# JonasFrey96/Visual-Odom-Pipeline

Measured on AMD Instinct MI355X. Metric: frames/sec @1241x376, 2000 KLT pts, 10-frame BA window, higher is better.
Workload: dtype u8/i32 (KLT, Shi-Tomasi) + f64 (DLT, BA); 1 GPU; kitti_shaped_1241x376_2000pts_ba10; sequences_per_gpu=256, batched_contexts_per_gpu=1, distinct_image_sequences=8, tracked_points=jittered grid (SURVEY 8d's fallback), launch=plain, solves_stopped_by_cap=0, solves_cut_and_rerun=0

## Files before the change

include/vo_mi355x.h:

```cpp
#ifndef VO_MI355X_H
#define VO_MI355X_H

#include <stdint.h>

#ifdef __cplusplus
extern "C" {
#endif

#define VO_ABI_VERSION 4

enum {
  VO_OK = 0,
  VO_E_INVALID = -1,
  VO_E_HIP = -2,
  VO_E_NOMEM = -3,
  VO_E_STATE = -4,
  VO_E_CAPACITY = -5,
  VO_E_NUMERIC = -6
};

typedef struct vo_ctx vo_ctx;


typedef struct {
// ... 395 lines not shown
  int32_t ba_landmarks, ba_observations, ba_iters, ba_accepted, ba_status, ba_done;
  int32_t t_final;
  double  ba_cost0, ba_cost;
  double  H[12];
  double  H_final[12];
} vo_pipe_record;

enum { VO_PIPE_LOST = 1, VO_PIPE_CAPACITY = 2, VO_PIPE_GROUPS = 4 };
enum { VO_PIPE_TRACK = 1, VO_PIPE_POSE = 2, VO_PIPE_TRIANGULATE = 4, VO_PIPE_ADJUST = 8, VO_PIPE_DETECT = 16, VO_PIPE_ALL = 31,
       VO_PIPE_TRACK_CANDIDATES = 32, VO_PIPE_TRACK_LANDMARKS = 64,
       VO_PIPE_KEEP_FREE_LISTS = 128 };
#define VO_PIPE_INFLIGHT 4
#define VO_PIPE_HIST 32

enum { VO_PIPE_K_TFIRST = 0, VO_PIPE_K_TTOTAL, VO_PIPE_K_HISTLEN, VO_PIPE_K_UV, VO_PIPE_K_UVFIRST, VO_PIPE_K_HIST, VO_PIPE_L_TLATEST,
       VO_PIPE_L_P, VO_PIPE_CAND, VO_PIPE_LM_L, VO_PIPE_LM_K, VO_PIPE_LM_KSHARED, VO_PIPE_DEAD_L, VO_PIPE_DEAD_K, VO_PIPE_COUNTS,
       VO_PIPE_POSES, VO_PIPE_N_TABLES };

int32_t vo_pipe_default_params(vo_pipe_params* p);
int32_t vo_pipe_create(vo_ctx* ctx, const double* K, const vo_pipe_params* prm);
int32_t vo_pipe_table_bytes(vo_ctx* ctx, int32_t which, uint64_t* bytes);
int32_t vo_pipe_table_write(vo_ctx* ctx, int32_t which, const void* src);
int32_t vo_pipe_table_read(vo_ctx* ctx, int32_t which, void* dst);
int32_t vo_pipe_commit(vo_ctx* ctx);
int32_t vo_pipe_step(vo_ctx* ctx, int32_t frame_idx, int32_t stages);
int32_t vo_pipe_step_host(vo_ctx* ctx, const uint8_t* const* frames, int32_t stride, int32_t stages);
int32_t vo_pipe_fetch(vo_ctx* ctx, vo_pipe_record* rec );
int32_t vo_pipe_set_ba_budget(vo_ctx* ctx, int32_t budget);
int32_t vo_pipe_lists_bytes(vo_ctx* ctx, uint64_t* bytes);
int32_t vo_pipe_lists_read(vo_ctx* ctx, void* dst);
int32_t vo_pipe_rows_read(vo_ctx* ctx, int32_t kind, const int32_t* rows, int32_t n, void* out);
int32_t vo_pipe_inliers_read(vo_ctx* ctx, uint8_t* mask, int32_t n);

typedef struct {
  int32_t ba_kernels;
  int32_t ba_lanes;
  int32_t ba_threads;
  int32_t ba_pitch_pad;
  int32_t ba_chunks;
  int32_t ba_workgroups;
  int32_t ba_workgroup_cap;
  int32_t ba_fold;
  int32_t klt_waves;
  int32_t klt_pair;
  int32_t st_two_kernels;
  int32_t st_band_rows;
  int32_t st_separate_nms;
  int32_t st_keep_eig;
  int32_t st_host_limit;
  int32_t xcd_remap_off;
  int32_t gate_groups;
  int32_t reserve_cus;
  int32_t gather_workgroups;
  int32_t reserved[13];
} vo_tuning;
int32_t vo_get_tuning(vo_ctx* ctx, vo_tuning* out);
int32_t vo_set_tuning(vo_ctx* ctx, const vo_tuning* t);

int32_t vo_frame_step_resident(vo_ctx* ctx, int32_t frame_idx, int32_t n_pts, int32_t do_dlt, int32_t do_ba,
                               int32_t do_st, int32_t mask_radius, const vo_klt_params* klt,
                               const vo_st_params* st, const vo_ba_params* ba);
int32_t vo_frame_fetch(vo_ctx* ctx, int32_t n_pts, float* p, uint8_t* status, float* err, float* X4,
                       double* depth1, double* reproj, double* poses, double* points, vo_ba_stats* stats,
                       float* corners, int32_t* n_corners);
int32_t vo_frame_step_host(vo_ctx* ctx, const uint8_t* const* frames, int32_t stride, int32_t n_pts, int32_t do_dlt, int32_t do_ba,
                           int32_t do_st, int32_t mask_radius, const vo_klt_params* klt,
                           const vo_st_params* st, const vo_ba_params* ba);
int32_t vo_host_alloc(uint64_t bytes, void** out);
int32_t vo_host_free(void* p);
int32_t vo_set_graph_mode(vo_ctx* ctx, int32_t on);
int32_t vo_set_side_stream(vo_ctx* ctx, int32_t on);
int32_t vo_step_layout(vo_ctx* ctx, int32_t* layout, int32_t* gate_groups, int32_t* reserved_cus);

enum { VO_PROF_FRAME = 0, VO_PROF_KLT = 1, VO_PROF_ST = 2, VO_PROF_DLT = 3, VO_PROF_BA = 4, VO_PROF_CLAHE_LUT = 5, VO_PROF_CLAHE_APPLY = 6,
       VO_PROF_HOM_SOLVE = 7, VO_PROF_HOM_SCORE = 8, VO_PROF_HOM_SELECT = 9, VO_PROF_HOM_FINISH = 10, VO_PROF_ORB_PYRAMID = 11,
       VO_PROF_ORB_CANDIDATES = 12, VO_PROF_ORB_RETAIN = 13, VO_PROF_ORB_DESCRIBE = 14,
       VO_PROF_FUND_SOLVE = 15, VO_PROF_FUND_SCORE = 16, VO_PROF_FUND_SELECT = 17, VO_PROF_FUND_FINISH = 18,
       VO_PROF_GMATCH_FORWARD = 19, VO_PROF_GMATCH_REVERSE = 20, VO_PROF_GMATCH_ACCEPT = 21, VO_PROF_HPOSE = 22,
       VO_PROF_SIM3_SOLVE = 23, VO_PROF_SIM3_SCORE = 24, VO_PROF_SIM3_SELECT = 25, VO_PROF_SIM3_FINISH = 26,
       VO_PROF_COUNT = 27 };
int32_t vo_profile_enable(vo_ctx* ctx, int32_t region_mask);
int32_t vo_profile_read(vo_ctx* ctx, int32_t region, double* total_ms, int32_t* count);
int32_t vo_debug_cycles(vo_ctx* ctx, int32_t which, int64_t* out8);

#ifdef __cplusplus
}
#endif
#endif
```

visual-odom-pipeline_amd/csrc/vo_klt.hip:

```cpp
#include "vo_klt_lk.h"

#include <stdlib.h>
#include <string.h>

template <int WAVES>
__global__ void __launch_bounds__(64, WAVES) k_klt_track(klt_args A, const float* __restrict__ p0, float* __restrict__ p1,
                                                  uint8_t* __restrict__ status, float* __restrict__ err,
                                                  int32_t* __restrict__ iters, unsigned long long* __restrict__ dbg,
                                                  const int32_t* __restrict__ counts) {
  int pt = blockIdx.x, bseq = blockIdx.y;
  if (A.xcd_remap) {
    const unsigned id = blockIdx.y * gridDim.x + blockIdx.x;
    const unsigned q = id >> 3;
    bseq = (int)(id & 7u) + 8 * (int)(q / (unsigned)A.n);
    pt = (int)(q % (unsigned)A.n);
  }
  if (pt >= A.n) return;
  const int lane = threadIdx.x;
  if (iters) iters += (size_t)bseq * A.iters_seq;
  const bool dead = counts && pt >= counts[bseq];
  if (iters && lane < A.iters_stride && (dead || lane > A.top)) iters[pt * A.iters_stride + lane] = -1;
  if (dead) return;
  p0 = vo_seq(p0, A.slab_seq, bseq); p1 = vo_seq(p1, A.slab_seq, bseq);
  status = vo_seq(status, A.slab_seq, bseq); err = vo_seq(err, A.slab_seq, bseq);
// ... 241 lines not shown
  p->win = 31; p->max_level = 3; p->max_count = 30; p->epsilon = 0.03; p->min_eig_threshold = 1e-4f; p->_pad = 0;
  return VO_OK;
}

static float klt_min_eig_numerator(float thr, float c) {
  auto from_ord = [](int64_t k) {
    const uint32_t u = (k >= 0) ? (uint32_t)k : (0x80000000u | (uint32_t)(-k));
    float f; memcpy(&f, &u, 4); return f;
  };
  const int64_t inf = 0x7F800000ll;
  if (!(thr == thr)) return __builtin_nanf("");
  int64_t lo = -inf, hi = inf;
  { volatile float q = from_ord(lo) / c; if (q >= thr) return from_ord(lo); }
  { volatile float q = from_ord(hi) / c; if (!(q >= thr)) return from_ord(hi); }
  while (hi - lo > 1) {
    const int64_t mid = lo + (hi - lo) / 2;
    volatile float q = from_ord(mid) / c;
    if (q >= thr) hi = mid; else lo = mid;
  }
  return from_ord(hi);
}

int32_t vo_klt_make_args(vo_ctx* c, int n, const vo_klt_params* prm, klt_args& A) {
  VO_CHECK(c, c->n_pushed >= 2, VO_E_STATE, "need two pushed frames");
  VO_CHECK(c, n >= 0 && n <= c->max_pts, VO_E_CAPACITY, "n exceeds max_pts");
  VO_CHECK(c, prm && prm->win >= 3 && prm->win <= VO_MAX_WIN && (prm->win & 1), VO_E_INVALID, "win must be odd, 3..31");
  VO_CHECK(c, prm->max_level >= 0 && prm->max_level < VO_MAX_LEVELS, VO_E_INVALID, "bad max_level");
  if (n == 0) return VO_OK;
  const vo_frame& P = c->fr[c->cur ^ 1];
  const vo_frame& C = c->fr[c->cur];
  int top = 0;
  for (int l = 1; l <= c->top && l <= prm->max_level; l++) {
    if (c->lv[l].w <= prm->win || c->lv[l].h <= prm->win) break;
    top = l;
  }
  for (int l = 0; l <= top; l++) {
    A.lv[l].imgI = P.img[l]; A.lv[l].derI = reinterpret_cast<const uint32_t*>(P.der[l]); A.lv[l].imgJ = C.img[l];
    A.lv[l].seq_px = c->lvl_px[l];
    A.lv[l].w = c->lv[l].w; A.lv[l].h = c->lv[l].h; A.lv[l].pitch = c->lv[l].pitch;
  }
  A.top = top; A.win = prm->win;
  A.xcd_remap = (!c->tune.xcd_remap_off && c->batch % 8 == 0) ? 1 : 0;
  int mc = prm->max_count; if (mc < 0) mc = 0; if (mc > 100) mc = 100;
  double eps = prm->epsilon; if (eps < 0) eps = 0; if (eps > 10) eps = 10;
  A.max_count = mc; A.eps2 = eps * eps; A.n = n;
  A.min_eig_num = klt_min_eig_numerator(prm->min_eig_threshold, (float)(2 * prm->win * prm->win));
  A.eps_lo = (float)(A.eps2 * (1.0 - 1e-6)); A.eps_hi = (float)(A.eps2 * (1.0 + 1e-6));
  A.iters_stride = prm->max_level + 1;
  A.slab_seq = c->slab_seq; A.iters_seq = (size_t)c->max_pts * VO_MAX_LEVELS;
  c->iters_stride = A.iters_stride;
  return VO_OK;
}

static void klt_launch_plain(vo_ctx* c, const klt_launch_rows& L, const klt_args& A) {
  const int waves = c->tune.klt_waves > 0 ? c->tune.klt_waves : 6;
#define VO_KLT_LAUNCH(WV) hipLaunchKernelGGL(k_klt_track<WV>, dim3(L.n, c->batch), dim3(64), 0, L.q, A, L.p0, L.p1, L.status, L.err, c->d_iters, c->d_dbg, L.counts)
#ifdef VO_EXPERIMENTS
  const int pair = c->tune.klt_pair;
  if (pair) {
    const int npair = (L.n + 1) / 2;
#define VO_KLT_LAUNCH2(WV) hipLaunchKernelGGL(k_klt_track2<WV>, dim3(npair, c->batch), dim3(64), 0, L.q, A, L.p0, L.p1, L.status, L.err, c->d_iters, L.counts)
    if (pair == 3) VO_KLT_LAUNCH2(3); else if (pair == 5) VO_KLT_LAUNCH2(5); else VO_KLT_LAUNCH2(4);
#undef VO_KLT_LAUNCH2
  } else
#endif
  if (waves <= 4) VO_KLT_LAUNCH(4); else if (waves == 5) VO_KLT_LAUNCH(5); else VO_KLT_LAUNCH(6);
#undef VO_KLT_LAUNCH
}

int32_t vo_klt_enqueue(vo_ctx* c, hipStream_t q, int n, const vo_klt_params* prm, size_t off_in, size_t off_out, const int32_t* d_counts, unsigned form) {
  const bool fb = form & KLT_FORM_FB, seeded = form & KLT_FORM_SEEDED;
  c->fb.n = -1;
  c->guess.n = -1;
  klt_args A;
  { const int32_t r = vo_klt_make_args(c, n, prm, A); if (r != VO_OK) return r; }
  if (n == 0) { if (fb) c->fb.n = 0; return VO_OK; }
  if (seeded) VO_CHECK(c, c->guess.d, VO_E_STATE, "no guesses");
  klt_fb_args F;
  if (fb) {
    { const int32_t r = vo_fb_reserve(c); if (r != VO_OK) return r; }
    vo_klt_fb_make_args(c, A, F);
  }
  const klt_launch_rows L = {q, n, vo_slab<const float>(c, off_in), vo_slab<float>(c, off_out), vo_slab<uint8_t>(c, c->off_status),
                        vo_slab<float>(c, c->off_err), d_counts};
  {
    vo_prof_scope prof(c, q, VO_PROF_KLT);
    if (seeded) vo_klt_launch_seeded(c, L, A, fb ? &F : nullptr);
    else if (fb) vo_klt_launch_fb(c, L, A, F);
    else klt_launch_plain(c, L, A);
  }
  VO_HIP(c, hipGetLastError());
  if (fb) c->fb.n = n;
  return VO_OK;
}

static int32_t klt_track_sync(vo_ctx* c, unsigned form, const float* p0, const float* guess, int32_t n, const vo_klt_params* prm, float* p1,
                              uint8_t* status, float* err, float* p0r, float* fb_err, int32_t* iters) {
  if (!c) return VO_E_INVALID;
  const bool fb = form & KLT_FORM_FB, seeded = form & KLT_FORM_SEEDED;
  vo_klt_params def;
  if (!prm) { vo_klt_default_params(&def); prm = &def; }
  VO_CHECK(c, n >= 0 && n <= c->max_pts, VO_E_CAPACITY, "n exceeds max_pts");
  if (n == 0) return VO_OK;
  VO_CHECK(c, p0 && p1 && status && err && (!fb || (p0r && fb_err)), VO_E_INVALID, "null buffer");
  VO_HIP(c, hipSetDevice(c->device));
  { const int32_t rq = vo_quiesce_side(c); if (rq != VO_OK) return rq; }
  if (seeded) { const int32_t rg = vo_guess_reserve(c); if (rg != VO_OK) return rg; }
// ... 81 lines not shown
```

visual-odom-pipeline_amd/csrc/vo_klt_lk.h:

```cpp
#pragma once
#include "vo_internal.h"

#define W_BITS 14

struct klt_level_args {
  const uint8_t* imgI;
  const uint32_t* derI;
  const uint8_t* imgJ;
  size_t seq_px;
  int w, h, pitch;
};

struct klt_args {
  klt_level_args lv[VO_MAX_LEVELS];
  size_t slab_seq;
  size_t iters_seq;
  int top, win, max_count, n, iters_stride;
  int xcd_remap;
  float min_eig_num;
  float eps_lo, eps_hi;
  double eps2;
};

struct klt_fb_args {
  klt_level_args bw[VO_MAX_LEVELS];
  size_t fb_seq;
  size_t off_err, off_ok;
  float max_err;
};

typedef uint32_t u32x3 __attribute__((ext_vector_type(3)));
__device__ __forceinline__ __amdgpu_buffer_rsrc_t klt_rsrc(const void* base) {
  return __builtin_amdgcn_make_buffer_rsrc(const_cast<void*>(base), 0, -1, 0x00020000);
}

__device__ __forceinline__ uint32_t row_next(uint32_t v, int lane) {
  return (uint32_t)__builtin_amdgcn_ds_bpermute(((lane + 16) & 63) << 2, (int)v);
}

__device__ __forceinline__ int wave_sum_i32(int v) {
  v += __builtin_amdgcn_update_dpp(0, v, 0x111 , 0xf, 0xf, false);
  v += __builtin_amdgcn_update_dpp(0, v, 0x112 , 0xf, 0xf, false);
  v += __builtin_amdgcn_update_dpp(0, v, 0x114 , 0xf, 0xf, false);
  v += __builtin_amdgcn_update_dpp(0, v, 0x118 , 0xf, 0xf, false);
  v += __builtin_amdgcn_update_dpp(0, v, 0x142 , 0xa, 0xf, false);
  v += __builtin_amdgcn_update_dpp(0, v, 0x143 , 0xc, 0xf, false);
  return __builtin_amdgcn_readlane(v, 63);
}

__device__ __forceinline__ float wave_sum_exact_f32(int v) {
  const int lo = wave_sum_i32(v & 0xFFFF);
  const int hi = wave_sum_i32(v >> 16);
  return (float)((double)hi * 65536.0 + (double)lo);
}
// ... 52 lines not shown
  const int w1 = klt_rows_sum(z >> 16);
  la = __builtin_amdgcn_readlane(w0, 0); lb = __builtin_amdgcn_readlane(w0, 1);
  lc = __builtin_amdgcn_readlane(w0, 2); hc = __builtin_amdgcn_readlane(w0, 3);
  ha = __builtin_amdgcn_readlane(w1, 0); hb = __builtin_amdgcn_readlane(w1, 1);
}

__device__ __forceinline__ float klt_combine(int hi, int lo) {
  if ((unsigned)(hi + 16384) < 32768u) return (float)(hi * 65536 + lo);
  return (float)((double)hi * 65536.0 + (double)lo);
}

__device__ __forceinline__ int klt_round(float x) { return __float_as_int(x + 12582912.f) - 0x4B400000; }

__device__ __forceinline__ void lk_weights(float a, float b, uint32_t& wt, uint32_t& wb) {
  const uint32_t r00 = (uint32_t)__float_as_int((1.f - a) * (1.f - b) * (float)(1 << W_BITS) + 12582912.f);
  const uint32_t r01 = (uint32_t)__float_as_int(a * (1.f - b) * (float)(1 << W_BITS) + 12582912.f);
  const uint32_t r10 = (uint32_t)__float_as_int((1.f - a) * b * (float)(1 << W_BITS) + 12582912.f);
  const uint32_t iw11 = (uint32_t)(1 << W_BITS) + 3u * 0x4B400000u - (r00 + r01 + r10);
  wt = __builtin_amdgcn_perm(r01, r00, 0x05040100u);
  wb = __builtin_amdgcn_perm(iw11, r10, 0x05040100u);
}

__device__ __forceinline__ float uniform_f(float v) {
  return __int_as_float(__builtin_amdgcn_readfirstlane(__float_as_int(v)));
}

typedef short s16x2 __attribute__((ext_vector_type(2)));

__device__ __forceinline__ int dot2(uint32_t a, uint32_t b, int c) {
  return __builtin_amdgcn_sdot2(__builtin_bit_cast(s16x2, a), __builtin_bit_cast(s16x2, b), c, false);
}
__device__ __forceinline__ int dot2k(uint32_t a, uint32_t b, int c) {
  return __builtin_amdgcn_sdot2(__builtin_bit_cast(s16x2, a), __builtin_bit_cast(s16x2, b), c, true);
}
__device__ __forceinline__ uint32_t pack_lo(uint32_t a, uint32_t b) { return __builtin_amdgcn_perm(b, a, 0x05040100u); }
__device__ __forceinline__ uint32_t pack_hi(uint32_t a, uint32_t b) { return __builtin_amdgcn_perm(b, a, 0x07060302u); }
__device__ __forceinline__ uint32_t bytes01(uint32_t t) { return __builtin_amdgcn_perm(0u, t, 0x0c010c00u); }
__device__ __forceinline__ uint32_t bytes12(uint32_t t) { return __builtin_amdgcn_perm(0u, t, 0x0c020c01u); }
__device__ __forceinline__ uint32_t pk_sub(uint32_t a, uint32_t b) {
  return __builtin_bit_cast(uint32_t, __builtin_bit_cast(s16x2, a) - __builtin_bit_cast(s16x2, b));
}
__device__ __forceinline__ uint32_t pk_abs(uint32_t a) {
  const s16x2 v = __builtin_bit_cast(s16x2, a);
  return __builtin_bit_cast(uint32_t, __builtin_elementwise_max(v, -v));
}

__device__ __forceinline__ uint32_t sample2(uint32_t T, uint32_t B, uint32_t wt, uint32_t wb) {
  const int s0 = dot2(bytes01(B), wb, dot2k(bytes01(T), wt, 1 << (W_BITS - 5 - 1)));
  const int s1 = dot2(bytes12(B), wb, dot2k(bytes12(T), wt, 1 << (W_BITS - 5 - 1)));
  typedef unsigned short u16x2 __attribute__((ext_vector_type(2)));
  const u16x2 h = __builtin_bit_cast(u16x2, __builtin_amdgcn_perm((uint32_t)s1, (uint32_t)s0, 0x06050201u));
  return __builtin_bit_cast(uint32_t, h >> (unsigned short)(W_BITS - 5 - 8));
}

__device__ __forceinline__ uint32_t deriv1(uint32_t top, uint32_t bot, uint32_t wt, uint32_t wb) {
  return (uint32_t)dot2(bot, wb, dot2k(top, wt, 1 << (W_BITS + 1)));
}

template <bool SEEDED = false>
__device__ __forceinline__ void klt_lk_point(const klt_args& A, const klt_level_args (&lv)[VO_MAX_LEVELS], int bseq, int pt, int lane,
                                             float p0x, float p0y, int32_t* iters, unsigned long long* dbgk,
                                             float& outx, float& outy, int& st, float& errv, float gx = 0.f, float gy = 0.f) {
  VO_STAMP(dbgk, 0);
  const int cp = lane & 15, r = lane >> 4;
  const int win = A.win;
  const float half = (float)(win - 1) * 0.5f;
  const float FLT_SCALE = 1.f / (float)(1 << 20);

  outx = 0.f; outy = 0.f;
  st = 1;
  errv = 0.f;

  const uint32_t colmask = ((2 * cp < win) ? 0x0000FFFFu : 0u) | ((2 * cp + 1 < win) ? 0xFFFF0000u : 0u);
  const uint32_t colones = colmask & 0x00010001u;
  const uint32_t colsel = (0x07060302u & colmask) | (0x0c0c0c0cu & ~colmask);

  for (int level = A.top; level >= 0; level--) {
    klt_level_args L = lv[level];
    L.imgI += (size_t)bseq * L.seq_px; L.derI += (size_t)bseq * L.seq_px; L.imgJ += (size_t)bseq * L.seq_px;
    const float scale = __int_as_float((127 - level) << 23);
    float prevx = p0x * scale, prevy = p0y * scale;
    float nextx, nexty;
    if (level == A.top) {
      if (SEEDED) { nextx = gx * scale; nexty = gy * scale; }
      else { nextx = prevx; nexty = prevy; }
    }
    else { nextx = outx * 2.f; nexty = outy * 2.f; }
    outx = nextx; outy = nexty;
    int n_it = -1;

    prevx -= half; prevy -= half;
    const float fpx = floorf(prevx), fpy = floorf(prevy);
    const int ipx = (int)fpx, ipy = (int)fpy;
    if (ipx < -win || ipx >= L.w || ipy < -win || ipy >= L.h) {
      if (level == 0) { st = 0; errv = 0.f; }
      if (iters && lane == 0) iters[pt * A.iters_stride + level] = n_it;
      continue;
    }
    const uint32_t lane_off = (uint32_t)(8 * r * L.pitch + 2 * cp);
    uint32_t wt, wb;
    lk_weights(prevx - fpx, prevy - fpy, wt, wb);

    uint32_t tI[8], tX[8], tY[8];
    {
      uint32_t T[8], D0[8], D1[8], D2[8];
      const uint32_t uo = (uint32_t)(ipy + VO_PAD) * (uint32_t)L.pitch + (uint32_t)(ipx + VO_PAD);
      const __amdgpu_buffer_rsrc_t rI = klt_rsrc(L.imgI), rD = klt_rsrc(L.derI);
#pragma unroll
      for (int s = 0; s < 8; s++) {
        const uint32_t o = uo + (uint32_t)s * (uint32_t)L.pitch;
        T[s] = __builtin_amdgcn_raw_buffer_load_b32(rI, (int)lane_off, (int)o, 0);
        const u32x3 d3 = __builtin_amdgcn_raw_buffer_load_b96(rD, (int)(lane_off * 4u), (int)(o * 4u), 0);
        D0[s] = d3[0]; D1[s] = d3[1]; D2[s] = d3[2];
      }
      const uint32_t T8 = row_next(T[0], lane), D08 = row_next(D0[0], lane), D18 = row_next(D1[0], lane), D28 = row_next(D2[0], lane);
      int a11 = 0, a12 = 0, a22 = 0;
#pragma unroll
      for (int s = 0; s < 8; s++) {
        const uint32_t B = (s < 7) ? T[(s + 1) & 7] : T8;
        const uint32_t E0 = (s < 7) ? D0[(s + 1) & 7] : D08;
        const uint32_t E1 = (s < 7) ? D1[(s + 1) & 7] : D18;
        const uint32_t E2 = (s < 7) ? D2[(s + 1) & 7] : D28;
        tI[s] = sample2(T[s], B, wt, wb);
        const uint32_t x0 = deriv1(pack_lo(D0[s], D1[s]), pack_lo(E0, E1), wt, wb);
        const uint32_t y0 = deriv1(pack_hi(D0[s], D1[s]), pack_hi(E0, E1), wt, wb);
        const uint32_t x1 = deriv1(pack_lo(D1[s], D2[s]), pack_lo(E1, E2), wt, wb);
        const uint32_t y1 = deriv1(pack_hi(D1[s], D2[s]), pack_hi(E1, E2), wt, wb);
        const uint32_t sel = (8 * r + s < win) ? colsel : 0x0c0c0c0cu;
        const uint32_t xp = __builtin_amdgcn_perm(x1, x0, sel), yp = __builtin_amdgcn_perm(y1, y0, sel);
        tX[s] = xp; tY[s] = yp;
        a11 = s ? dot2(xp, xp, a11) : dot2k(xp, xp, 0);
        a12 = s ? dot2(xp, yp, a12) : dot2k(xp, yp, 0);
        a22 = s ? dot2(yp, yp, a22) : dot2k(yp, yp, 0);
      }
      float A11, A12, A22;
      {
        int l11, h11, l12, h12, l22, h22;
        wave_sum3_wide(a11, a12, a22, lane, l11, h11, l12, h12, l22, h22);
        A11 = klt_combine(h11, l11) * FLT_SCALE; A12 = klt_combine(h12, l12) * FLT_SCALE; A22 = klt_combine(h22, l22) * FLT_SCALE;
      }
      if (level == A.top) VO_STAMP(dbgk, 1);
      float D = A11 * A22 - A12 * A12;
      const float num = A22 + A11 - sqrtf((A11 - A22) * (A11 - A22) + 4.f * A12 * A12);
      if (num < A.min_eig_num || D < 1.1920929e-07f) {
        if (level == 0) st = 0;
        if (iters && lane == 0) iters[pt * A.iters_stride + level] = n_it;
        continue;
      }
      D = 1.f / D;

      nextx -= half; nexty -= half;
      const __amdgpu_buffer_rsrc_t rJ = klt_rsrc(L.imgJ);
      float pdx = 0.f, pdy = 0.f;
      int j = 0;
      for (; j < A.max_count; j++) {
        const float fnx = floorf(nextx), fny = floorf(nexty);
        const int inx = (int)fnx, iny = (int)fny;
        if (inx < -win || inx >= L.w || iny < -win || iny >= L.h) {
          if (level == 0) st = 0;
          break;
        }
        uint32_t jt, jb;
        lk_weights(nextx - fnx, nexty - fny, jt, jb);
        uint32_t Tj[8];
        const uint32_t uj = (uint32_t)(iny + VO_PAD) * (uint32_t)L.pitch + (uint32_t)(inx + VO_PAD);
#pragma unroll
        for (int s = 0; s < 8; s++) Tj[s] = __builtin_amdgcn_raw_buffer_load_b32(rJ, (int)lane_off, (int)(uj + (uint32_t)s * (uint32_t)L.pitch), 0);
        const uint32_t Tj8 = row_next(Tj[0], lane);
        int b1 = 0, b2 = 0;
#pragma unroll
        for (int s = 0; s < 8; s++) {
          const uint32_t B = (s < 7) ? Tj[(s + 1) & 7] : Tj8;
          const uint32_t d = pk_sub(sample2(Tj[s], B, jt, jb), tI[s]);
          b1 = s ? dot2(d, tX[s], b1) : dot2k(d, tX[0], 0);
          b2 = s ? dot2(d, tY[s], b2) : dot2k(d, tY[0], 0);
        }
        int l1, h1, l2, h2;
        wave_sum2_wide(b1, b2, lane, l1, h1, l2, h2);
        const float fb1 = klt_combine(h1, l1) * FLT_SCALE;
        const float fb2 = klt_combine(h2, l2) * FLT_SCALE;
        const float dx = (A12 * fb2 - A22 * fb1) * D;
        const float dy = (A12 * fb1 - A11 * fb2) * D;
        nextx += dx; nexty += dy;
        outx = nextx + half; outy = nexty + half;
        const float d2 = dx * dx + dy * dy;
        bool conv;
        if (d2 < A.eps_lo) conv = true;
        else if (d2 > A.eps_hi) conv = false;
        else conv = (double)dx * (double)dx + (double)dy * (double)dy <= A.eps2;
        if (conv) { j++; break; }
        if (j > 0 && fabsf(dx + pdx) <= 0.01f && fabsf(dy + pdy) <= 0.01f) {
          outx -= dx * 0.5f; outy -= dy * 0.5f;
          j++;
          break;
        }
        pdx = dx; pdy = dy;
        if (level == A.top && j == 0) VO_STAMP(dbgk, 2);
      }
      n_it = j;
      if (level == A.top) VO_STAMP(dbgk, 3);
      if (level == 1) VO_STAMP(dbgk, 4);
      if (iters && lane == 0) iters[pt * A.iters_stride + level] = n_it;

      if (st && level == 0) {
        const float nx = outx - half, ny = outy - half;
        const float fnx = floorf(nx), fny = floorf(ny);
        const int inx = (int)fnx, iny = (int)fny;
        if (inx < -win || inx >= L.w || iny < -win || iny >= L.h) {
          st = 0;
        } else {
          uint32_t jt, jb;
          lk_weights(nx - fnx, ny - fny, jt, jb);
          uint32_t Tj[8];
          const uint32_t uj = (uint32_t)(iny + VO_PAD) * (uint32_t)L.pitch + (uint32_t)(inx + VO_PAD);
#pragma unroll
          for (int s = 0; s < 8; s++) Tj[s] = __builtin_amdgcn_raw_buffer_load_b32(rJ, (int)lane_off, (int)(uj + (uint32_t)s * (uint32_t)L.pitch), 0);
          const uint32_t Tj8 = row_next(Tj[0], lane);
          int e = 0;
#pragma unroll
          for (int s = 0; s < 8; s++) {
            const uint32_t B = (s < 7) ? Tj[(s + 1) & 7] : Tj8;
            const uint32_t d = pk_abs(pk_sub(sample2(Tj[s], B, jt, jb), tI[s]));
            const uint32_t ones = (8 * r + s < win) ? colones : 0u;
            e = s ? dot2(d, ones, e) : dot2k(d, ones, 0);
          }
          const int ierr = wave_sum_i32(e);
          errv = (float)ierr * 1.f / (float)(32 * win * win);
        }
      }
    }
  }
  VO_STAMP(dbgk, 5);
}

int32_t vo_klt_enqueue(vo_ctx* c, hipStream_t q, int n, const vo_klt_params* prm, size_t off_in, size_t off_out, const int32_t* d_counts, unsigned form);
int32_t vo_klt_make_args(vo_ctx* c, int n, const vo_klt_params* prm, klt_args& A);
void vo_klt_fb_make_args(const vo_ctx* c, const klt_args& A, klt_fb_args& F);

struct klt_launch_rows {
  hipStream_t q;
  int n;
  const float* p0; float* p1; uint8_t* status; float* err;
  const int32_t* counts;
};
void vo_klt_launch_fb(vo_ctx* c, const klt_launch_rows& L, const klt_args& A, const klt_fb_args& F);
void vo_klt_launch_seeded(vo_ctx* c, const klt_launch_rows& L, const klt_args& A, const klt_fb_args* F);

inline hipError_t iters_d2h(vo_ctx* c, int32_t* h, int n, int levels) {
  return rows_d2h(c, h, c->d_iters, sizeof(int32_t) * (size_t)c->max_pts * VO_MAX_LEVELS, sizeof(int32_t) * (size_t)n * levels);
}
```

visual-odom-pipeline_amd/csrc/vo_step.hip:

```cpp
#include "vo_internal.h"

#include <stdlib.h>
#include <string.h>

#include <mutex>
#include <vector>
#include <stdio.h>
static std::mutex g_trace_mu;
static std::vector<hipEvent_t> g_tr, g_ta, g_tb;
static void trace_push(std::vector<hipEvent_t>& v, hipStream_t st, size_t cap) {
  std::lock_guard<std::mutex> lk(g_trace_mu);
  if (v.size() >= cap) return;
  hipEvent_t e;
  if (hipEventCreate(&e) != hipSuccess) return;
  (void)hipEventRecord(e, st);
  v.push_back(e);
}
extern "C" void vo_debug_step_trace_dump(int first_step, int n_steps) {
  std::lock_guard<std::mutex> lk(g_trace_mu);
  for (size_t i = 2 * (size_t)(first_step < 0 ? 0 : first_step); i + 3 < g_tr.size() && i + 3 < g_ta.size() && i + 3 < g_tb.size() && i < 2 * (size_t)(first_step + n_steps); i += 2) {
    float d = 0, gap = 0, a0 = 0, a1 = 0;
    (void)hipEventElapsedTime(&d, g_tr[i], g_tr[i + 1]);
    (void)hipEventElapsedTime(&gap, g_tr[i + 1], g_tr[i + 2]);
    (void)hipEventElapsedTime(&a0, g_tr[i], g_ta[i + 2]);
// ... 392 lines not shown
    if (c->tune.gate_groups) groups = c->tune.gate_groups > 0 ? c->tune.gate_groups : 0;
    if (c->tune.reserve_cus) reserve = c->tune.reserve_cus > 0 ? c->tune.reserve_cus : 0;
  }
  c->ba_wide_groups = groups;
  c->ba_wide_recorded = false;
  c->layout_suspended = false;
  return vo_main_stream_reserve(c, reserve);
}

static int32_t pipelined_setup(vo_ctx* c) {
  hipEvent_t (*const pairs[4])[2] = {&c->ev_ba_wide, &c->ev_ba, &c->ev_pub, &c->ev_copy1};
  hipStream_t st = nullptr; hipEvent_t ev[8] = {};
  VO_HIP(c, hipSetDevice(c->device));
  hipError_t e = hipStreamCreateWithFlags(&st, hipStreamNonBlocking);
  for (int i = 0; i < 8 && e == hipSuccess; i++) e = hipEventCreateWithFlags(&ev[i], hipEventDisableTiming);
  if (e != hipSuccess) {
    for (hipEvent_t x : ev) if (x) (void)hipEventDestroy(x);
    if (st) (void)hipStreamDestroy(st);
    VO_HIP(c, e);
  }
  for (int i = 0; i < 8; i++) (*pairs[i / 2])[i % 2] = ev[i];
  c->stream3 = st;
  return VO_OK;
}

extern "C" int32_t vo_set_side_stream(vo_ctx* c, int32_t on) {
  if (!c) return VO_E_INVALID;
  VO_CHECK(c, c->steps_enq == c->steps_fetched && !vo_pipe_busy(c), VO_E_STATE, "fetch the steps in flight before switching the stream layout");
  if (on == 2 && !c->stream3) { const int32_t rs = pipelined_setup(c); if (rs != VO_OK) return rs; }
  c->side_stream = (on == 2) ? 2 : (on ? 1 : 0);
  return step_layout_apply(c);
}

extern "C" int32_t vo_get_tuning(vo_ctx* c, vo_tuning* out) {
  if (!c || !out) return VO_E_INVALID;
  *out = c->tune;
  return VO_OK;
}

extern "C" int32_t vo_set_tuning(vo_ctx* c, const vo_tuning* t) {
  if (!c || !t) return VO_E_INVALID;
  VO_CHECK(c, c->steps_enq == c->steps_fetched && !vo_pipe_busy(c), VO_E_STATE, "fetch the steps in flight before changing the tuning");
  VO_CHECK(c, (t->ba_kernels >= 0 && t->ba_kernels <= 2) && (t->ba_lanes == 0 || t->ba_lanes == 8 || t->ba_lanes == 16) &&
              (t->ba_threads == 0 || t->ba_threads == 256 || t->ba_threads == 512 || t->ba_threads == 1024) && t->ba_pitch_pad >= 0 && t->ba_pitch_pad <= 64 &&
              t->ba_chunks >= 0 && t->ba_workgroups >= 0 && t->ba_workgroup_cap >= 0 && t->ba_fold >= 0 && t->ba_fold <= 2 &&
              (t->klt_waves == 0 || (t->klt_waves >= 4 && t->klt_waves <= 6)) && t->st_band_rows >= 0 && t->gate_groups >= -1 && t->reserve_cus >= -1 &&
              t->reserve_cus < 256, VO_E_INVALID, "field out of range");
#ifndef VO_EXPERIMENTS
  VO_CHECK(c, t->klt_pair == 0, VO_E_INVALID, "klt_pair needs a build with -DVO_EXPERIMENTS");
#else
  VO_CHECK(c, t->klt_pair == 0 || (t->klt_pair >= 3 && t->klt_pair <= 5), VO_E_INVALID, "klt_pair: 3, 4 or 5");
#endif
  VO_CHECK(c, t->gather_workgroups >= 0 && t->gather_workgroups <= 65536, VO_E_INVALID, "gather_workgroups out of range");
  for (int k = 0; k < 13; k++) VO_CHECK(c, t->reserved[k] == 0, VO_E_INVALID, "reserved fields must be 0");
  VO_HIP(c, hipSetDevice(c->device));
  { const int32_t rq = vo_quiesce_side(c); if (rq != VO_OK) return rq; }
  c->tune = *t;
  for (auto& g : c->step_graphs) if (g.second) (void)hipGraphExecDestroy(g.second);
  c->step_graphs.clear();
  return step_layout_apply(c);
}

extern "C" int32_t vo_step_layout(vo_ctx* c, int32_t* layout, int32_t* gate_groups, int32_t* reserved_cus) {
  if (!c) return VO_E_INVALID;
  if (layout) *layout = c->side_stream;
  if (gate_groups) *gate_groups = c->ba_wide_groups;
  if (reserved_cus) *reserved_cus = c->stream_reserve;
  return VO_OK;
}

extern "C" int32_t vo_set_graph_mode(vo_ctx* c, int32_t on) {
  if (!c) return VO_E_INVALID;
  VO_CHECK(c, c->steps_enq == c->steps_fetched && !vo_pipe_busy(c), VO_E_STATE, "fetch the steps in flight before switching the launch mode");
  c->use_graph = on ? 1 : 0;
  { const int32_t rr = step_layout_apply(c); if (rr != VO_OK) return rr; }
  return VO_OK;
}
```

visual-odom-pipeline_amd/vo_mi355x/_lib.py:

```python
import ctypes as C
import os

import numpy as np

_HERE = os.path.dirname(os.path.abspath(__file__))
PKG_ROOT = os.path.dirname(_HERE)
LIB_PATH = os.environ.get("VO_MI355X_LIB") or os.path.join(PKG_ROOT, "lib", "libvo_mi355x.so")
CSRC_DIR = os.path.join(PKG_ROOT, "csrc")

VO_OK = 0
ERRORS = {-1: "VO_E_INVALID", -2: "VO_E_HIP", -3: "VO_E_NOMEM", -4: "VO_E_STATE", -5: "VO_E_CAPACITY",
          -6: "VO_E_NUMERIC"}


class VoError(RuntimeError):
    def __init__(self, code, msg):
        super().__init__("%s (%d): %s" % (ERRORS.get(code, "VO_E_?"), code, msg))
        self.code = code


class KltParams(C.Structure):
    _fields_ = [("win", C.c_int32), ("max_level", C.c_int32), ("max_count", C.c_int32),
                ("epsilon", C.c_double), ("min_eig_threshold", C.c_float), ("_pad", C.c_int32)]


class SubpixParams(C.Structure):
    _fields_ = [("win_x", C.c_int32), ("win_y", C.c_int32), ("zero_x", C.c_int32), ("zero_y", C.c_int32), ("max_count", C.c_int32),
                ("_pad", C.c_int32), ("epsilon", C.c_double)]


class BriefParams(C.Structure):
    _fields_ = [("n_bits", C.c_int32), ("_pad", C.c_int32), ("reserved", C.c_int32 * 6)]


class StParams(C.Structure):
    _fields_ = [("max_corners", C.c_int32), ("block_size", C.c_int32), ("quality_level", C.c_double),
                ("min_distance", C.c_double), ("use_harris", C.c_int32), ("fast_threshold", C.c_int32), ("harris_k", C.c_double)]


LOSSES = {"huber": 0, "linear": 1, "soft_l1": 2, "cauchy": 3, "arctan": 4}


def loss_code(loss):
    if callable(loss):
        raise NotImplementedError("a callable loss is not supported by the HIP bundle adjustment; use one of %s" % sorted(LOSSES))
    if loss not in LOSSES:
        raise ValueError("loss must be one of %s, got %r" % (sorted(LOSSES), loss))
    return LOSSES[loss]


class BaParams(C.Structure):
    _fields_ = [("max_iters", C.c_int32), ("loss", C.c_int32), ("ftol", C.c_double), ("xtol", C.c_double),
                ("gtol", C.c_double), ("lambda0", C.c_double), ("huber_delta", C.c_double), ("lambda_min", C.c_double)]


TUNING_FIELDS = ("ba_kernels", "ba_lanes", "ba_threads", "ba_pitch_pad", "ba_chunks", "ba_workgroups", "ba_workgroup_cap", "ba_fold", "klt_waves", "klt_pair",
                 "st_two_kernels", "st_band_rows", "st_separate_nms", "st_keep_eig", "st_host_limit", "xcd_remap_off", "gate_groups", "reserve_cus",
                 "gather_workgroups")


class Tuning(C.Structure):
    _fields_ = [(k, C.c_int32) for k in TUNING_FIELDS] + [("reserved", C.c_int32 * 13)]


class PnpParams(C.Structure):
    _fields_ = [("reproj_err", C.c_double), ("confidence", C.c_double), ("max_iters", C.c_int32), ("seed", C.c_int32)]


class PnpStats(C.Structure):
    _fields_ = [("cost", C.c_double), ("n_inliers", C.c_int32), ("hypotheses", C.c_int32), ("best", C.c_int32),
                ("status", C.c_int32)]


class EssParams(C.Structure):
    _fields_ = [("threshold", C.c_double), ("prob", C.c_double), ("distance_thresh", C.c_double), ("max_iters", C.c_int32),
                ("seed", C.c_int32)]


class EssStats(C.Structure):
    _fields_ = [("n_inliers", C.c_int32), ("n_good", C.c_int32), ("hypotheses", C.c_int32), ("best", C.c_int32),
                ("status", C.c_int32), ("_pad", C.c_int32)]


class HomParams(C.Structure):
    _fields_ = [("threshold", C.c_double), ("confidence", C.c_double), ("max_iters", C.c_int32), ("seed", C.c_int32),
                ("refine_iters", C.c_int32), ("_pad", C.c_int32)]


class HomStats(C.Structure):
    _fields_ = [("cost", C.c_double), ("n_inliers", C.c_int32), ("hypotheses", C.c_int32), ("best", C.c_int32),
                ("status", C.c_int32), ("lm_iters", C.c_int32), ("_pad", C.c_int32)]


class FundParams(C.Structure):
    _fields_ = [("threshold", C.c_double), ("confidence", C.c_double), ("max_iters", C.c_int32), ("seed", C.c_int32),
                ("refit", C.c_int32), ("_pad", C.c_int32)]


class FundStats(C.Structure):
    _fields_ = [("cost", C.c_double), ("n_inliers", C.c_int32), ("hypotheses", C.c_int32), ("best", C.c_int32),
                ("status", C.c_int32), ("n_roots", C.c_int32), ("models", C.c_int32)]


class Sim3Params(C.Structure):
    _fields_ = [("threshold", C.c_double), ("confidence", C.c_double), ("max_iters", C.c_int32), ("seed", C.c_int32),
                ("with_scale", C.c_int32), ("refit", C.c_int32)]


class Sim3Stats(C.Structure):
    _fields_ = [("cost", C.c_double), ("n_inliers", C.c_int32), ("hypotheses", C.c_int32), ("best", C.c_int32),
                ("status", C.c_int32), ("degenerate", C.c_int32), ("refit", C.c_int32)]


class HposeParams(C.Structure):
    _fields_ = [("ratio", C.c_double), ("threshold", C.c_double), ("hint", C.c_double * 3), ("min_off", C.c_int32), ("use_hint", C.c_int32)]
# ... 234 lines not shown
```

Before: 47600 frames/s.

## Cache KLT target-window rows in LDS across iterations within same integer cell

Adds a KLT tracking kernel variant that gathers the 9 rows of the target image window into LDS as byte-pair expansions and reuses them across Lucas-Kanade iterations while the integer patch position stays unchanged. Global buffer loads are reissued only when the wave-uniform cell changes. The variant is on by default through a tuning field when no wave or pair override is set. It is meant to cut repeated global loads and byte unpacking per iteration, at the cost of LDS traffic, a shared buffer per block, and asm pins that constrain scheduling.

Result: faster. 49240 frames/s (median of 6 runs) (+3.4%).

```diff
diff --git a/include/vo_mi355x.h b/include/vo_mi355x.h
--- a/include/vo_mi355x.h
+++ b/include/vo_mi355x.h
@@ -471,7 +471,8 @@
   int32_t gate_groups;
   int32_t reserve_cus;
   int32_t gather_workgroups;
-  int32_t reserved[13];
+  int32_t klt_reuse;
+  int32_t reserved[12];
 } vo_tuning;
 int32_t vo_get_tuning(vo_ctx* ctx, vo_tuning* out);
 int32_t vo_set_tuning(vo_ctx* ctx, const vo_tuning* t);
diff --git a/visual-odom-pipeline_amd/csrc/vo_klt.hip b/visual-odom-pipeline_amd/csrc/vo_klt.hip
--- a/visual-odom-pipeline_amd/csrc/vo_klt.hip
+++ b/visual-odom-pipeline_amd/csrc/vo_klt.hip
@@ -317,7 +317,10 @@
   return VO_OK;
 }
 
+#define KLT_REUSE_RULE 1
 static void klt_launch_plain(vo_ctx* c, const klt_launch_rows& L, const klt_args& A) {
+  const bool rule = KLT_REUSE_RULE && c->tune.klt_waves == 0 && c->tune.klt_pair == 0;
+  if (c->tune.klt_reuse > 0 || (c->tune.klt_reuse == 0 && rule)) { vo_klt_launch_reuse(c, L, A); return; }
   const int waves = c->tune.klt_waves > 0 ? c->tune.klt_waves : 6;
 #define VO_KLT_LAUNCH(WV) hipLaunchKernelGGL(k_klt_track<WV>, dim3(L.n, c->batch), dim3(64), 0, L.q, A, L.p0, L.p1, L.status, L.err, c->d_iters, c->d_dbg, L.counts)
 #ifdef VO_EXPERIMENTS
diff --git a/visual-odom-pipeline_amd/csrc/vo_klt_lk.h b/visual-odom-pipeline_amd/csrc/vo_klt_lk.h
--- a/visual-odom-pipeline_amd/csrc/vo_klt_lk.h
+++ b/visual-odom-pipeline_amd/csrc/vo_klt_lk.h
@@ -1,5 +1,7 @@
 #pragma once
 #include "vo_internal.h"
+
+#include <limits.h>
 
 #define W_BITS 14
 
@@ -158,12 +160,40 @@
   const u16x2 h = __builtin_bit_cast(u16x2, __builtin_amdgcn_perm((uint32_t)s1, (uint32_t)s0, 0x06050201u));
   return __builtin_bit_cast(uint32_t, h >> (unsigned short)(W_BITS - 5 - 8));
 }
+__device__ __forceinline__ uint2 sample2_gather(uint32_t T) { return make_uint2(bytes01(T), bytes12(T)); }
+__device__ __forceinline__ uint32_t sample2_combine(uint2 t, uint2 b, uint32_t wt, uint32_t wb) {
+  const int s0 = dot2(b.x, wb, dot2k(t.x, wt, 1 << (W_BITS - 5 - 1)));
+  const int s1 = dot2(b.y, wb, dot2k(t.y, wt, 1 << (W_BITS - 5 - 1)));
+  typedef unsigned short u16x2 __attribute__((ext_vector_type(2)));
+  const u16x2 h = __builtin_bit_cast(u16x2, __builtin_amdgcn_perm((uint32_t)s1, (uint32_t)s0, 0x06050201u));
+  return __builtin_bit_cast(uint32_t, h >> (unsigned short)(W_BITS - 5 - 8));
+}
+
+__device__ __forceinline__ char* klt_rows_lds() {
+  __shared__ uint2 rows[9 * 64];
+  return reinterpret_cast<char*>(rows);
+}
+__device__ __forceinline__ uint2 klt_row_read(const char* rows, uint32_t ab, int k) {
+  return *reinterpret_cast<const uint2*>(rows + ab + (uint32_t)k * 512u);
+}
+__device__ __forceinline__ void klt_rows_fetch(char* rows, uint32_t ab, __amdgpu_buffer_rsrc_t rJ, uint32_t lane_off, uint32_t uo, uint32_t pitch, int lane) {
+  uint32_t Tj[8];
+#pragma unroll
+  for (int s = 0; s < 8; s++) Tj[s] = __builtin_amdgcn_raw_buffer_load_b32(rJ, (int)lane_off, (int)(uo + (uint32_t)s * pitch), 0);
+  const uint32_t Tj8 = row_next(Tj[0], lane);
+#pragma unroll
+  for (int k = 0; k < 9; k++) {
+    *reinterpret_cast<uint2*>(rows + ab + (uint32_t)k * 512u) = sample2_gather(k < 8 ? Tj[k & 7] : Tj8);
+  }
+}
+#define KLT_ROWS_PIN(ab, acc) asm volatile("" : "+v"(ab), "+v"(acc))
+#define KLT_ROWS_OPAQUE(v) asm volatile("" : "+v"(v))
 
 __device__ __forceinline__ uint32_t deriv1(uint32_t top, uint32_t bot, uint32_t wt, uint32_t wb) {
   return (uint32_t)dot2(bot, wb, dot2k(top, wt, 1 << (W_BITS + 1)));
 }
 
-template <bool SEEDED = false>
+template <bool SEEDED = false, bool REUSE = false>
 __device__ __forceinline__ void klt_lk_point(const klt_args& A, const klt_level_args (&lv)[VO_MAX_LEVELS], int bseq, int pt, int lane,
                                              float p0x, float p0y, int32_t* iters, unsigned long long* dbgk,
                                              float& outx, float& outy, int& st, float& errv, float gx = 0.f, float gy = 0.f) {
@@ -180,6 +210,9 @@
   const uint32_t colmask = ((2 * cp < win) ? 0x0000FFFFu : 0u) | ((2 * cp + 1 < win) ? 0xFFFF0000u : 0u);
   const uint32_t colones = colmask & 0x00010001u;
   const uint32_t colsel = (0x07060302u & colmask) | (0x0c0c0c0cu & ~colmask);
+  char* rows = nullptr;
+  uint32_t rows_ab = 0;
+  if constexpr (REUSE) { rows = klt_rows_lds(); rows_ab = (uint32_t)lane * 8u; }
 
   for (int level = A.top; level >= 0; level--) {
     klt_level_args L = lv[level];
@@ -258,6 +291,7 @@
       nextx -= half; nexty -= half;
       const __amdgpu_buffer_rsrc_t rJ = klt_rsrc(L.imgJ);
       float pdx = 0.f, pdy = 0.f;
+      int cellx = INT_MIN, celly = INT_MIN;
       int j = 0;
       for (; j < A.max_count; j++) {
         const float fnx = floorf(nextx), fny = floorf(nexty);
@@ -268,18 +302,38 @@
         }
         uint32_t jt, jb;
         lk_weights(nextx - fnx, nexty - fny, jt, jb);
-        uint32_t Tj[8];
-        const uint32_t uj = (uint32_t)(iny + VO_PAD) * (uint32_t)L.pitch + (uint32_t)(inx + VO_PAD);
-#pragma unroll
-        for (int s = 0; s < 8; s++) Tj[s] = __builtin_amdgcn_raw_buffer_load_b32(rJ, (int)lane_off, (int)(uj + (uint32_t)s * (uint32_t)L.pitch), 0);
-        const uint32_t Tj8 = row_next(Tj[0], lane);
         int b1 = 0, b2 = 0;
-#pragma unroll
-        for (int s = 0; s < 8; s++) {
-          const uint32_t B = (s < 7) ? Tj[(s + 1) & 7] : Tj8;
-          const uint32_t d = pk_sub(sample2(Tj[s], B, jt, jb), tI[s]);
-          b1 = s ? dot2(d, tX[s], b1) : dot2k(d, tX[0], 0);
-          b2 = s ? dot2(d, tY[s], b2) : dot2k(d, tY[0], 0);
+        if constexpr (REUSE) {
+          const int ux = __builtin_amdgcn_readfirstlane(inx), uy = __builtin_amdgcn_readfirstlane(iny);
+          if (ux != cellx || uy != celly) {
+            klt_rows_fetch(rows, rows_ab, rJ, lane_off, (uint32_t)(uy + VO_PAD) * (uint32_t)L.pitch + (uint32_t)(ux + VO_PAD), (uint32_t)L.pitch, lane);
+            cellx = ux; celly = uy;
+          }
+          KLT_ROWS_OPAQUE(rows_ab);
+          uint2 r0 = klt_row_read(rows, rows_ab, 0), r1 = klt_row_read(rows, rows_ab, 1);
+#pragma unroll
+          for (int s = 0; s < 8; s++) {
+            uint2 r2 = r1;
+            if (s < 7) r2 = klt_row_read(rows, rows_ab, s + 2);
+            const uint32_t d = pk_sub(sample2_combine(r0, r1, jt, jb), tI[s]);
+            b1 = s ? dot2(d, tX[s], b1) : dot2k(d, tX[0], 0);
+            b2 = s ? dot2(d, tY[s], b2) : dot2k(d, tY[0], 0);
+            if (s < 6) KLT_ROWS_PIN(rows_ab, b1);
+            r0 = r1; r1 = r2;
+          }
+        } else {
+          uint32_t Tj[8];
+          const uint32_t uj = (uint32_t)(iny + VO_PAD) * (uint32_t)L.pitch + (uint32_t)(inx + VO_PAD);
+#pragma unroll
+          for (int s = 0; s < 8; s++) Tj[s] = __builtin_amdgcn_raw_buffer_load_b32(rJ, (int)lane_off, (int)(uj + (uint32_t)s * (uint32_t)L.pitch), 0);
+          const uint32_t Tj8 = row_next(Tj[0], lane);
+#pragma unroll
+          for (int s = 0; s < 8; s++) {
+            const uint32_t B = (s < 7) ? Tj[(s + 1) & 7] : Tj8;
+            const uint32_t d = pk_sub(sample2(Tj[s], B, jt, jb), tI[s]);
+            b1 = s ? dot2(d, tX[s], b1) : dot2k(d, tX[0], 0);
+            b2 = s ? dot2(d, tY[s], b2) : dot2k(d, tY[0], 0);
+          }
         }
         int l1, h1, l2, h2;
         wave_sum2_wide(b1, b2, lane, l1, h1, l2, h2);
@@ -317,18 +371,38 @@
         } else {
           uint32_t jt, jb;
           lk_weights(nx - fnx, ny - fny, jt, jb);
-          uint32_t Tj[8];
-          const uint32_t uj = (uint32_t)(iny + VO_PAD) * (uint32_t)L.pitch + (uint32_t)(inx + VO_PAD);
-#pragma unroll
-          for (int s = 0; s < 8; s++) Tj[s] = __builtin_amdgcn_raw_buffer_load_b32(rJ, (int)lane_off, (int)(uj + (uint32_t)s * (uint32_t)L.pitch), 0);
-          const uint32_t Tj8 = row_next(Tj[0], lane);
           int e = 0;
-#pragma unroll
-          for (int s = 0; s < 8; s++) {
-            const uint32_t B = (s < 7) ? Tj[(s + 1) & 7] : Tj8;
-            const uint32_t d = pk_abs(pk_sub(sample2(Tj[s], B, jt, jb), tI[s]));
-            const uint32_t ones = (8 * r + s < win) ? colones : 0u;
-            e = s ? dot2(d, ones, e) : dot2k(d, ones, 0);
+          if constexpr (REUSE) {
+            const int ux = __builtin_amdgcn_readfirstlane(inx), uy = __builtin_amdgcn_readfirstlane(iny);
+            if (ux != cellx || uy != celly)
+              klt_rows_fetch(rows, rows_ab, rJ, lane_off, (uint32_t)(uy + VO_PAD) * (uint32_t)L.pitch + (uint32_t)(ux + VO_PAD), (uint32_t)L.pitch, lane);
+            KLT_ROWS_OPAQUE(rows_ab);
+            uint32_t cones = colones;
+            KLT_ROWS_OPAQUE(cones);
+            uint2 r0 = klt_row_read(rows, rows_ab, 0), r1 = klt_row_read(rows, rows_ab, 1);
+#pragma unroll
+            for (int s = 0; s < 8; s++) {
+              uint2 r2 = r1;
+              if (s < 7) r2 = klt_row_read(rows, rows_ab, s + 2);
+              const uint32_t d = pk_abs(pk_sub(sample2_combine(r0, r1, jt, jb), tI[s]));
+              const uint32_t ones = (8 * r + s < win) ? cones : 0u;
+              e = s ? dot2(d, ones, e) : dot2k(d, ones, 0);
+              if (s < 6) KLT_ROWS_PIN(rows_ab, e);
+              r0 = r1; r1 = r2;
+            }
+          } else {
+            uint32_t Tj[8];
+            const uint32_t uj = (uint32_t)(iny + VO_PAD) * (uint32_t)L.pitch + (uint32_t)(inx + VO_PAD);
+#pragma unroll
+            for (int s = 0; s < 8; s++) Tj[s] = __builtin_amdgcn_raw_buffer_load_b32(rJ, (int)lane_off, (int)(uj + (uint32_t)s * (uint32_t)L.pitch), 0);
+            const uint32_t Tj8 = row_next(Tj[0], lane);
+#pragma unroll
+            for (int s = 0; s < 8; s++) {
+              const uint32_t B = (s < 7) ? Tj[(s + 1) & 7] : Tj8;
+              const uint32_t d = pk_abs(pk_sub(sample2(Tj[s], B, jt, jb), tI[s]));
+              const uint32_t ones = (8 * r + s < win) ? colones : 0u;
+              e = s ? dot2(d, ones, e) : dot2k(d, ones, 0);
+            }
           }
           const int ierr = wave_sum_i32(e);
           errv = (float)ierr * 1.f / (float)(32 * win * win);
@@ -351,6 +425,7 @@
 };
 void vo_klt_launch_fb(vo_ctx* c, const klt_launch_rows& L, const klt_args& A, const klt_fb_args& F);
 void vo_klt_launch_seeded(vo_ctx* c, const klt_launch_rows& L, const klt_args& A, const klt_fb_args* F);
+void vo_klt_launch_reuse(vo_ctx* c, const klt_launch_rows& L, const klt_args& A);
 
 inline hipError_t iters_d2h(vo_ctx* c, int32_t* h, int n, int levels) {
   return rows_d2h(c, h, c->d_iters, sizeof(int32_t) * (size_t)c->max_pts * VO_MAX_LEVELS, sizeof(int32_t) * (size_t)n * levels);
diff --git a/visual-odom-pipeline_amd/csrc/vo_klt_reuse.hip b/visual-odom-pipeline_amd/csrc/vo_klt_reuse.hip
--- /dev/null
+++ b/visual-odom-pipeline_amd/csrc/vo_klt_reuse.hip
@@ -0,0 +1,37 @@
+#include "vo_klt_lk.h"
+
+template <int WAVES>
+__global__ void __launch_bounds__(64, WAVES) k_klt_track_r(klt_args A, const float* __restrict__ p0, float* __restrict__ p1,
+                                                    uint8_t* __restrict__ status, float* __restrict__ err,
+                                                    int32_t* __restrict__ iters, unsigned long long* __restrict__ dbg,
+                                                    const int32_t* __restrict__ counts) {
+  int pt = blockIdx.x, bseq = blockIdx.y;
+  if (A.xcd_remap) {
+    const unsigned id = blockIdx.y * gridDim.x + blockIdx.x;
+    const unsigned q = id >> 3;
+    bseq = (int)(id & 7u) + 8 * (int)(q / (unsigned)A.n);
+    pt = (int)(q % (unsigned)A.n);
+  }
+  if (pt >= A.n) return;
+  const int lane = threadIdx.x;
+  if (iters) iters += (size_t)bseq * A.iters_seq;
+  const bool dead = counts && pt >= counts[bseq];
+  if (iters && lane < A.iters_stride && (dead || lane > A.top)) iters[pt * A.iters_stride + lane] = -1;
+  if (dead) return;
+  p0 = vo_seq(p0, A.slab_seq, bseq); p1 = vo_seq(p1, A.slab_seq, bseq);
+  status = vo_seq(status, A.slab_seq, bseq); err = vo_seq(err, A.slab_seq, bseq);
+  unsigned long long* dbgk = (pt == A.n / 2 && bseq == 0 && dbg) ? dbg + 24 : nullptr;
+  const float p0x = uniform_f(p0[2 * pt]), p0y = uniform_f(p0[2 * pt + 1]);
+  float outx, outy, errv;
+  int st;
+  klt_lk_point<false, true>(A, A.lv, bseq, pt, lane, p0x, p0y, iters, dbgk, outx, outy, st, errv);
+  if (lane == 0) {
+    p1[2 * pt] = outx; p1[2 * pt + 1] = outy;
+    status[pt] = (uint8_t)st;
+    err[pt] = st ? errv : 0.f;
+  }
+}
+
+void vo_klt_launch_reuse(vo_ctx* c, const klt_launch_rows& L, const klt_args& A) {
+  hipLaunchKernelGGL(k_klt_track_r<6>, dim3(L.n, c->batch), dim3(64), 0, L.q, A, L.p0, L.p1, L.status, L.err, c->d_iters, c->d_dbg, L.counts);
+}
diff --git a/visual-odom-pipeline_amd/csrc/vo_step.hip b/visual-odom-pipeline_amd/csrc/vo_step.hip
--- a/visual-odom-pipeline_amd/csrc/vo_step.hip
+++ b/visual-odom-pipeline_amd/csrc/vo_step.hip
@@ -468,7 +468,8 @@
   VO_CHECK(c, t->klt_pair == 0 || (t->klt_pair >= 3 && t->klt_pair <= 5), VO_E_INVALID, "klt_pair: 3, 4 or 5");
 #endif
   VO_CHECK(c, t->gather_workgroups >= 0 && t->gather_workgroups <= 65536, VO_E_INVALID, "gather_workgroups out of range");
-  for (int k = 0; k < 13; k++) VO_CHECK(c, t->reserved[k] == 0, VO_E_INVALID, "reserved fields must be 0");
+  VO_CHECK(c, t->klt_reuse >= -1 && t->klt_reuse <= 1, VO_E_INVALID, "klt_reuse: -1, 0 or 1");
+  for (int k = 0; k < 12; k++) VO_CHECK(c, t->reserved[k] == 0, VO_E_INVALID, "reserved fields must be 0");
   VO_HIP(c, hipSetDevice(c->device));
   { const int32_t rq = vo_quiesce_side(c); if (rq != VO_OK) return rq; }
   c->tune = *t;
diff --git a/visual-odom-pipeline_amd/vo_mi355x/_lib.py b/visual-odom-pipeline_amd/vo_mi355x/_lib.py
--- a/visual-odom-pipeline_amd/vo_mi355x/_lib.py
+++ b/visual-odom-pipeline_amd/vo_mi355x/_lib.py
@@ -56,11 +56,11 @@
 
 TUNING_FIELDS = ("ba_kernels", "ba_lanes", "ba_threads", "ba_pitch_pad", "ba_chunks", "ba_workgroups", "ba_workgroup_cap", "ba_fold", "klt_waves", "klt_pair",
                  "st_two_kernels", "st_band_rows", "st_separate_nms", "st_keep_eig", "st_host_limit", "xcd_remap_off", "gate_groups", "reserve_cus",
-                 "gather_workgroups")
+                 "gather_workgroups", "klt_reuse")
 
 
 class Tuning(C.Structure):
-    _fields_ = [(k, C.c_int32) for k in TUNING_FIELDS] + [("reserved", C.c_int32 * 13)]
+    _fields_ = [(k, C.c_int32) for k in TUNING_FIELDS] + [("reserved", C.c_int32 * 12)]
 
 
 class PnpParams(C.Structure):
```
